# jlk9/MPAS-Ocean.jl

Measured on AMD Instinct MI355X. Metric: cell-updates/sec per RK4 step, higher is better.
Workload: dtype f64

## Files before the change

include/moka_hip.h:

```cpp
#ifndef MOKA_HIP_H
#define MOKA_HIP_H
#include <stdint.h>

#ifdef __cplusplus
extern "C" {
#endif

typedef struct moka_ctx   moka_ctx;
typedef struct moka_plan  moka_plan;
typedef struct moka_mesh  moka_mesh;
typedef struct moka_state moka_state;

typedef enum {
    MOKA_OK = 0,
    MOKA_ERR_ARG = -1,
    MOKA_ERR_HIP = -2,
    MOKA_ERR_NO_DEVICE = -3,
    MOKA_ERR_ALLOC = -4,
    MOKA_ERR_UNSUPPORTED = -5,
    MOKA_ERR_COMM = -6
} moka_status;

typedef enum {
    MOKA_ORDER_DEFAULT = 0,
    MOKA_ORDER_NONE = 1,
    MOKA_ORDER_RCM = 2,
    MOKA_ORDER_RCB = 3
} moka_ordering;

typedef struct moka_mesh_desc {
    int32_t nCells, nEdges, nVertices;
    int32_t maxEdges, maxEdges2, vertexDegree;
    int32_t nVertLevels;
    int32_t edgeSignOnVertexLD;
    const double  *xCell, *yCell, *zCell;
    const int32_t *nEdgesOnCell;
    const int32_t *edgesOnCell;
    const int32_t *edgeSignOnCell;
    const double  *areaCell;
    const int32_t *cellsOnEdge;
    const int32_t *verticesOnEdge;
    const int32_t *nEdgesOnEdge;
    const int32_t *edgesOnEdge;
    const double  *weightsOnEdge;
    const double  *dvEdge, *dcEdge, *fEdge;
    const int32_t *edgesOnVertex;
    const int32_t *cellsOnVertex;
    const int32_t *edgeSignOnVertex;
    const double  *areaTriangle;
    const int32_t *maxLevelEdgeTop;
    const double  *restingThicknessSum;
    int32_t ordering;
    int32_t patch_cells;
    const int32_t *cellClass;
    int32_t stateBytes;
    const double *kiteAreasOnVertex;
    const double *fVertex;
} moka_mesh_desc;

typedef struct moka_mesh_info {
    int32_t nCells, nEdges, nVertices, nVertLevels;
    int32_t ordering, patch_cells, nPatches;
    int32_t maxEdgesUsed, maxEdges2Used;
    int32_t lanesPerColumn;
    int64_t meshBytesDevice;
    int64_t cellBandwidth;
    int32_t maxPatchRows;
    int32_t ldsBytesPerBlock;
    int32_t maxPatchCells, maxPatchEdges;
} moka_mesh_info;

enum { MOKA_CELL = 0, MOKA_EDGE = 1, MOKA_VERTEX = 2 };

typedef enum {
    MOKA_F_SSH = 0,
    MOKA_F_NORMAL_VELOCITY = 1,
    MOKA_F_LAYER_THICKNESS = 2,
    MOKA_F_LAYER_THICKNESS_EDGE = 3,
    MOKA_F_THICKNESS_FLUX = 4,
    MOKA_F_VELOCITY_DIV_CELL = 5,
    MOKA_F_RELATIVE_VORTICITY = 6,
    MOKA_F_TEND_NORMAL_VELOCITY = 7,
    MOKA_F_TEND_LAYER_THICKNESS = 8
} moka_field;

#define MOKA_FE_STALE_HEDGE      1
#define MOKA_FE_ACCUM_VORT       2
#define MOKA_FE_LEVEL1_ONLY      4
#define MOKA_FE_REFERENCE_COMPAT 7

typedef enum { MOKA_FORWARD_EULER = 0, MOKA_RUNGE_KUTTA_4 = 1 } moka_integrator;

const char *moka_version(void);
int  moka_ctx_create(int device, moka_ctx **out);
void moka_ctx_destroy(moka_ctx *ctx);
const char *moka_last_error(const moka_ctx *ctx);
int  moka_sync(moka_ctx *ctx);
int  moka_timer_start(moka_ctx *ctx);
int  moka_timer_stop(moka_ctx *ctx, float *elapsed_ms);

int  moka_plan_create(const moka_mesh_desc *desc, moka_plan **out);
void moka_plan_destroy(moka_plan *plan);
int  moka_plan_info(const moka_plan *plan, moka_mesh_info *info);
int  moka_plan_permutation(const moka_plan *plan, int kind, int32_t *new_to_old);
int  moka_plan_patch_ranges(const moka_plan *plan, int32_t *cellStart, int32_t *edgeStart, int32_t *vertexStart);
int  moka_plan_class_ranges(const moka_plan *plan, int32_t capacity, int32_t *nClasses, int32_t *patchStart,
                            int32_t *cellStart, int32_t *edgeStart);

enum {
    MOKA_PA_EOC = 0, MOKA_PA_COC, MOKA_PA_MLTC, MOKA_PA_SDV, MOKA_PA_INVAREA, MOKA_PA_AREACELL, MOKA_PA_RSUM,
    MOKA_PA_EHDR, MOKA_PA_EOE, MOKA_PA_WOE, MOKA_PA_GINVDC, MOKA_PA_DCEDGE, MOKA_PA_DVEDGE, MOKA_PA_FEDGE,
    MOKA_PA_EOV, MOKA_PA_CV, MOKA_PA_HALO_START, MOKA_PA_HALO_EDGE, MOKA_PA_LEOC, MOKA_PA_LEOE,
    MOKA_PA_CREC, MOKA_PA_EREC, MOKA_PA_FEOE, MOKA_PA_PVSTART, MOKA_PA_PVLIST, MOKA_PA_LVOE
};
int  moka_plan_array(const moka_plan *plan, int which, const void **data, int64_t *count);

int  moka_mesh_create(moka_ctx *ctx, const moka_mesh_desc *desc, moka_mesh **out);
void moka_mesh_destroy(moka_mesh *mesh);
int  moka_mesh_info_get(const moka_mesh *mesh, moka_mesh_info *info);

int moka_gradient_on_edge(moka_mesh *mesh, const double *scalarCell, double *gradEdge);
int moka_divergence_on_cell(moka_mesh *mesh, const double *vecEdge, double *tempEdge, double *divCell);
int moka_curl_on_vertex(moka_mesh *mesh, const double *vecEdge, double *curlVertex);
int moka_interpolate_cell2edge(moka_mesh *mesh, const double *cellValue, double *edgeValue, int nlev);

int moka_gradient_on_edge_vjp(moka_mesh *mesh, double *dGradEdge , double *dScalarCell );
int moka_gradient_on_edge_jvp(moka_mesh *mesh, const double *dScalarCell, double *dGradEdge);
int moka_divergence_on_cell_vjp(moka_mesh *mesh, double *dDivCell , double *dVecEdge ,
                                double *dTempEdge );
int moka_divergence_on_cell_jvp(moka_mesh *mesh, const double *dVecEdge, double *dTempEdge , double *dDivCell);
int moka_curl_on_vertex_vjp(moka_mesh *mesh, const double *dCurlVertex, double *dVecEdge );
int moka_curl_on_vertex_jvp(moka_mesh *mesh, const double *dVecEdge, double *dCurlVertex );

int  moka_state_create(moka_ctx *ctx, moka_mesh *mesh, moka_state **out);
void moka_state_destroy(moka_state *st);
int  moka_state_upload(moka_state *st, int field, int time_level, const double *host);
int  moka_state_download(moka_state *st, int field, int time_level, double *host);

int  moka_state_download_rows(moka_state *st, int field, int time_level, int64_t nRows, const int32_t *rows, double *host);

int  moka_state_array_address(moka_state *st, int field, int time_level, uint64_t *address);

int  moka_state_optimize_placement(moka_state *st, int max_tries, double *ms_before, double *ms_after);
typedef struct { int32_t field; double ms_old, ms_new; int32_t kept; } moka_placement_trial;
int  moka_state_placement_log(const moka_state *st, int32_t capacity, moka_placement_trial *out, int32_t *n);
int64_t moka_state_placement_launches(const moka_state *st);

int moka_advance_time_levels(moka_state *st, int flags);
int moka_diagnostic_compute(moka_state *st, int flags);
int moka_compute_normal_velocity_tendency(moka_state *st, int flags);
int moka_compute_layer_thickness_tendency(moka_state *st, int flags);
int moka_tendencies(moka_state *st);
int moka_step_fe(moka_state *st, double dt, int flags);
int moka_step_rk4(moka_state *st, double dt);
int moka_run(moka_state *st, int integrator, double dt, int64_t nsteps, int flags);
int moka_sum_sq(moka_state *st, int field, int time_level, double *out);

typedef struct moka_halo moka_halo;
int  moka_ctx_streams(moka_ctx *ctx, void **compute_stream, void **comm_stream);
int  moka_mesh_permutation(const moka_mesh *mesh, int kind, int32_t *new_to_old);
int  moka_mesh_class_ranges(const moka_mesh *mesh, int32_t capacity, int32_t *nClasses, int32_t *patchStart,
                            int32_t *cellStart, int32_t *edgeStart);
int  moka_halo_create(moka_state *st, int32_t nNeighbors, const int32_t *sendCells, const int64_t *sendCellOff,
                      const int32_t *sendEdges, const int64_t *sendEdgeOff, const int32_t *recvCells,
                      const int64_t *recvCellOff, const int32_t *recvEdges, const int64_t *recvEdgeOff,
                      int32_t nPatchesBoundary, int32_t nPatchesOwned, moka_halo **out);
void moka_halo_destroy(moka_halo *h);
int  moka_halo_buffer_elems(const moka_halo *h, int64_t *sendElems, int64_t *recvElems);
int  moka_halo_pack(moka_halo *h, int what, void *sendbuf_device);
int  moka_halo_unpack(moka_halo *h, int what, const void *recvbuf_device);

typedef struct {
    unsigned char ipc[15][64];
    uint64_t ptr[15];
    uint64_t flagPtr;
    char     shmName[64];
    int32_t  dstCell, dstEdge;
    int32_t  nCells, nEdges;
    int32_t  slot;
    int32_t  nNeighbors, pid, device, stateBytes, nVertLevels;
// ... 104 lines not shown
```

mpas-ocean.jl_amd/csrc/plan.cpp:

```cpp
#include <algorithm>
#include <array>
#include <cmath>
#include <new>
#include <numeric>
#include <queue>

#include "moka_internal.hpp"

namespace moka {

static thread_local std::string g_err;
void set_error(const std::string &msg) { g_err = msg; }
const char *get_error() { return g_err.c_str(); }

namespace {

inline int64_t IX(int i, int64_t j, int ld) { return j * ld + i; }

#define REQUIRE(cond, msg)                 \
    do {                                   \
        if (!(cond)) {                     \
            set_error(msg);                \
            return MOKA_ERR_ARG;           \
        }                                  \
    } while (0)

std::vector<int> partition_by_class(const moka_mesh_desc *d, std::vector<int32_t> &n2o)
{
    std::vector<int> bounds{0};
    if (!d->cellClass) { bounds.push_back((int)n2o.size()); return bounds; }
    int maxc = 0;
    for (int c = 0; c < d->nCells; ++c) maxc = std::max(maxc, (int)d->cellClass[c]);
    std::vector<int32_t> out;
    out.reserve(n2o.size());
    for (int k = 0; k <= maxc; ++k) {
        for (int32_t c : n2o) if (d->cellClass[c] == k) out.push_back(c);
        bounds.push_back((int)out.size());
    }
    n2o.swap(out);
    return bounds;
}

void rcb_order(const moka_mesh_desc *d, int P, std::vector<int32_t> &n2o)
{
    const int n = d->nCells;
    n2o.resize(n);
    std::iota(n2o.begin(), n2o.end(), 0);
    const double *X[3] = {d->xCell, d->yCell, d->zCell};
    struct Range { int lo, hi; };
    std::vector<Range> stack;
    {
        const std::vector<int> b = partition_by_class(d, n2o);
        for (size_t i = b.size() - 1; i >= 1; --i) if (b[i] > b[i - 1]) stack.push_back({b[i - 1], b[i]});
    }
    while (!stack.empty()) {
        Range r = stack.back();
        stack.pop_back();
        const int cnt = r.hi - r.lo;
        if (cnt <= P) {
            continue;
        }
        int axis = 0;
        double best = -1.0;
        for (int a = 0; a < 3; ++a) {
            if (!X[a]) continue;
            double mn = 1e300, mx = -1e300;
            for (int i = r.lo; i < r.hi; ++i) {
                double v = X[a][n2o[i]];
                mn = std::min(mn, v);
                mx = std::max(mx, v);
            }
            if (mx - mn > best) { best = mx - mn; axis = a; }
        }
        const int leaves = (cnt + P - 1) / P;
        const int left = (leaves / 2) * P;
        const double *xa = X[axis];
        std::nth_element(n2o.begin() + r.lo, n2o.begin() + r.lo + left, n2o.begin() + r.hi,
                         [xa](int32_t a, int32_t b) { return xa[a] < xa[b] || (xa[a] == xa[b] && a < b); });
        stack.push_back({r.lo + left, r.hi});
        stack.push_back({r.lo, r.lo + left});
    }
}

void rcm_order(const moka_mesh_desc *d, std::vector<int32_t> &n2o)
{
    const int n = d->nCells;
    std::vector<int32_t> deg(n, 0), start(n + 1, 0), adj;
    for (int64_t e = 0; e < d->nEdges; ++e) {
        int a = d->cellsOnEdge[2 * e] - 1, b = d->cellsOnEdge[2 * e + 1] - 1;
        if (a >= 0 && b >= 0 && a != b) { ++deg[a]; ++deg[b]; }
    }
    for (int i = 0; i < n; ++i) start[i + 1] = start[i] + deg[i];
    adj.resize(start[n]);
    std::vector<int32_t> fill(start.begin(), start.end() - 1);
    for (int64_t e = 0; e < d->nEdges; ++e) {
        int a = d->cellsOnEdge[2 * e] - 1, b = d->cellsOnEdge[2 * e + 1] - 1;
        if (a >= 0 && b >= 0 && a != b) { adj[fill[a]++] = b; adj[fill[b]++] = a; }
    }
    std::vector<char> seen(n, 0);
    std::vector<int32_t> order;
    order.reserve(n);
    auto bfs_far = [&](int s, std::vector<int32_t> &lvl) {
        std::vector<int32_t> q{s};
        lvl.assign(n, -1);
        lvl[s] = 0;
        size_t h = 0;
        while (h < q.size()) {
            int u = q[h++];
            for (int k = start[u]; k < start[u + 1]; ++k)
                if (lvl[adj[k]] < 0 && !seen[adj[k]]) { lvl[adj[k]] = lvl[u] + 1; q.push_back(adj[k]); }
        }
        return q.back();
    };
    std::vector<int32_t> lvl;
    for (int s0 = 0; s0 < n; ++s0) {
        if (seen[s0]) continue;
        int s = bfs_far(bfs_far(s0, lvl), lvl);
        std::vector<int32_t> q{s};
        seen[s] = 1;
        size_t h = 0;
        std::vector<int32_t> nb;
        while (h < q.size()) {
            int u = q[h++];
            nb.clear();
            for (int k = start[u]; k < start[u + 1]; ++k)
                if (!seen[adj[k]]) { seen[adj[k]] = 1; nb.push_back(adj[k]); }
            std::sort(nb.begin(), nb.end(), [&](int a, int b) { return deg[a] < deg[b] || (deg[a] == deg[b] && a < b); });
            q.insert(q.end(), nb.begin(), nb.end());
        }
        order.insert(order.end(), q.begin(), q.end());
    }
    n2o.assign(order.rbegin(), order.rend());
}

}

int build_plan(const moka_mesh_desc *d, Plan &p)
{
    REQUIRE(d != nullptr, "mesh descriptor is NULL");
    REQUIRE(d->nCells > 0 && d->nEdges > 0 && d->nVertices > 0, "mesh counts must be positive");
    REQUIRE(d->nVertLevels >= 1, "nVertLevels must be >= 1");
    REQUIRE(d->maxEdges >= 3 && d->maxEdges2 >= 1 && d->vertexDegree >= 3, "bad maxEdges/maxEdges2/vertexDegree");
    REQUIRE(d->nEdgesOnCell && d->edgesOnCell && d->edgeSignOnCell && d->areaCell, "PrimaryCells arrays missing");
    REQUIRE(d->cellsOnEdge && d->nEdgesOnEdge && d->edgesOnEdge && d->weightsOnEdge && d->dvEdge && d->dcEdge && d->fEdge,
            "Edges arrays missing");
    REQUIRE(d->edgesOnVertex && d->edgeSignOnVertex && d->areaTriangle, "DualCells arrays missing");
    REQUIRE(d->restingThicknessSum, "restingThicknessSum missing");
    const int nC = d->nCells, nE = d->nEdges, nV = d->nVertices, VD = d->vertexDegree;
    const int ldSV = d->edgeSignOnVertexLD > 0 ? d->edgeSignOnVertexLD : VD;
    REQUIRE(ldSV >= VD, "edgeSignOnVertexLD < vertexDegree");

    int maxEoC = 0, maxEoE = 0;
    for (int c = 0; c < nC; ++c) {
        int n = d->nEdgesOnCell[c];
        REQUIRE(n >= 1 && n <= d->maxEdges, "nEdgesOnCell out of range");
        maxEoC = std::max(maxEoC, n);
        for (int i = 0; i < n; ++i) {
            int e = d->edgesOnCell[IX(i, c, d->maxEdges)];
            REQUIRE(e >= 1 && e <= nE, "edgesOnCell out of range");
            int s = d->edgeSignOnCell[IX(i, c, d->maxEdges)];
            REQUIRE(s == 1 || s == -1, "edgeSignOnCell must be +-1 on active slots");
        }
        REQUIRE(d->areaCell[c] > 0.0, "areaCell must be positive");
    }
    for (int e = 0; e < nE; ++e) {
        int a = d->cellsOnEdge[2 * (int64_t)e], b = d->cellsOnEdge[2 * (int64_t)e + 1];
        REQUIRE(a >= 1 && a <= nC && b >= 1 && b <= nC, "cellsOnEdge out of range (non-periodic meshes are not supported, VertMesh.jl:50)");
        int n = d->nEdgesOnEdge[e];
        REQUIRE(n >= 0 && n <= d->maxEdges2, "nEdgesOnEdge out of range");
        maxEoE = std::max(maxEoE, n);
        for (int i = 0; i < n; ++i) {
            int x = d->edgesOnEdge[IX(i, e, d->maxEdges2)];
            REQUIRE(x >= 0 && x <= nE, "edgesOnEdge out of range");
        }
        REQUIRE(d->dcEdge[e] > 0.0, "dcEdge must be positive");
        if (d->maxLevelEdgeTop) REQUIRE(d->maxLevelEdgeTop[e] >= 0 && d->maxLevelEdgeTop[e] <= d->nVertLevels, "maxLevelEdgeTop out of range");
    }
    for (int v = 0; v < nV; ++v) {
        for (int j = 0; j < VD; ++j) {
            int e = d->edgesOnVertex[IX(j, v, VD)];
            REQUIRE(e >= 1 && e <= nE, "edgesOnVertex out of range");
            int s = d->edgeSignOnVertex[IX(j, v, ldSV)];
            REQUIRE(s == 1 || s == -1, "edgeSignOnVertex must be +-1");
        }
        REQUIRE(d->areaTriangle[v] > 0.0, "areaTriangle must be positive");
    }

    p.nC = nC; p.nE = nE; p.nV = nV; p.K = d->nVertLevels; p.VD = VD;
    p.ME = maxEoC <= 6 ? 6 : (maxEoC <= 8 ? 8 : maxEoC);
    p.ME2 = maxEoE <= 10 ? 10 : (maxEoE <= 14 ? 14 : maxEoE);
    if (p.ME == 8 && p.ME2 < 14) p.ME2 = 14;
    {
        const int K = d->nVertLevels;
        REQUIRE(d->stateBytes == 0 || d->stateBytes == 4 || d->stateBytes == 8, "stateBytes must be 0, 4 or 8");
        p.stateBytes = d->stateBytes == 4 ? 4 : 8;
        int def = 32;
        if (p.stateBytes == 8 && K >= 34 && K <= 64 && !(K & 1)) def = 16;
        if (p.stateBytes == 4 && K >= 34 && K <= 128 && !(K & 3)) def = 24;
        p.P = d->patch_cells > 0 ? d->patch_cells : def;
    }
    REQUIRE(p.P <= 4096, "patch_cells too large");

    int ordering = d->ordering;
    const bool haveXYZ = d->xCell && d->yCell;
    if (ordering == MOKA_ORDER_DEFAULT) ordering = haveXYZ ? MOKA_ORDER_RCB : MOKA_ORDER_RCM;
    REQUIRE(ordering >= MOKA_ORDER_NONE && ordering <= MOKA_ORDER_RCB, "unknown ordering");
    REQUIRE(ordering != MOKA_ORDER_RCB || haveXYZ, "RCB ordering needs xCell/yCell");
    p.ordering = ordering;
    if (d->cellClass)
        for (int c = 0; c < nC; ++c) REQUIRE(d->cellClass[c] >= 0 && d->cellClass[c] < 64, "cellClass out of range");
    if (ordering == MOKA_ORDER_RCB) rcb_order(d, p.P, p.cellN2O);
    else if (ordering == MOKA_ORDER_RCM) { rcm_order(d, p.cellN2O); partition_by_class(d, p.cellN2O); }
    else { p.cellN2O.resize(nC); std::iota(p.cellN2O.begin(), p.cellN2O.end(), 0); partition_by_class(d, p.cellN2O); }
    p.cellO2N.assign(nC, -1);
    for (int i = 0; i < nC; ++i) p.cellO2N[p.cellN2O[i]] = i;

    std::vector<int32_t> patchOf(nC);
    p.classCellStart.assign(1, 0);
    p.classPatchStart.assign(1, 0);
    p.patchCellStart.assign(1, 0);
    {
        auto cls0 = [&](int cn) { return d->cellClass ? d->cellClass[p.cellN2O[cn]] : 0; };
        int begin = 0;
        while (begin < nC) {
            const int k = cls0(begin);
            int end = begin;
            while (end < nC && cls0(end) == k) ++end;
            REQUIRE((int)p.classCellStart.size() - 1 <= k, "internal: cell ordering is not class-major");
            while ((int)p.classCellStart.size() - 1 < k) {
                p.classCellStart.push_back(begin);
                p.classPatchStart.push_back((int)p.patchCellStart.size() - 1);
            }
            for (int c = begin; c < end; c += p.P) {
                const int q = (int)p.patchCellStart.size() - 1;
                for (int x = c; x < std::min(c + p.P, end); ++x) patchOf[x] = q;
                p.patchCellStart.push_back(std::min(c + p.P, end));
            }
            p.classCellStart.push_back(end);
            p.classPatchStart.push_back((int)p.patchCellStart.size() - 1);
            begin = end;
        }
    }
    p.nPatches = (int)p.patchCellStart.size() - 1;

    auto renumber = [&](int n, auto owner_of, std::vector<int32_t> &n2o, std::vector<int32_t> &o2n) {
        std::vector<int32_t> owner(n), cnt(nC + 1, 0);
        for (int i = 0; i < n; ++i) { owner[i] = owner_of(i); ++cnt[owner[i] + 1]; }
        for (int c = 0; c < nC; ++c) cnt[c + 1] += cnt[c];
        n2o.resize(n); o2n.resize(n);
        for (int i = 0; i < n; ++i) { int pos = cnt[owner[i]]++; n2o[pos] = i; o2n[i] = pos; }
        return owner;
    };
    std::vector<int32_t> ownerCell(nE);
    {
        const int P = p.P, nP = p.nPatches;
        std::vector<int32_t> cnt(nP, 0), flex;
        auto PO = [&](int cn) { return patchOf[cn]; };
        auto cls = [&](int cn) { return d->cellClass ? d->cellClass[p.cellN2O[cn]] : 0; };
        std::vector<int32_t> lo(nE), hi(nE);
        for (int e = 0; e < nE; ++e) {
            const int a = p.cellO2N[d->cellsOnEdge[2 * (int64_t)e] - 1], b = p.cellO2N[d->cellsOnEdge[2 * (int64_t)e + 1] - 1];
            lo[e] = std::min(a, b); hi[e] = std::max(a, b);
            if (PO(lo[e]) == PO(hi[e]) || cls(lo[e]) != cls(hi[e])) {
                ownerCell[e] = lo[e];
                ++cnt[PO(lo[e])];
            } else {
                ownerCell[e] = -1;
                flex.push_back(e);
            }
        }
        std::stable_sort(flex.begin(), flex.end(), [&](int x, int y) { return lo[x] < lo[y]; });
        for (int e : flex) {
            const int pa = PO(lo[e]), pb = PO(hi[e]);
            if (((uint32_t)e * 2654435761u >> 15) & 1u) { ownerCell[e] = lo[e]; ++cnt[pa]; }
            else { ownerCell[e] = hi[e]; ++cnt[pb]; }
        }
        for (int sweep = 0; sweep < 16; ++sweep) {
            int moved = 0;
            for (int e : flex) {
                const int cur = ownerCell[e], oth = cur == lo[e] ? hi[e] : lo[e];
                if (cnt[PO(cur)] > cnt[PO(oth)] + 1) { ownerCell[e] = oth; --cnt[PO(cur)]; ++cnt[PO(oth)]; ++moved; }
            }
            if (!moved) break;
        }
        {
            std::vector<int32_t> pcls(nP), Tc(64, 0);
            {
                std::vector<int64_t> tot(64, 0), num(64, 0);
                for (int q = 0; q < nP; ++q) {
                    pcls[q] = cls(p.patchCellStart[q]);
                    if (p.patchCellStart[q + 1] - p.patchCellStart[q] == P) { tot[pcls[q]] += cnt[q]; ++num[pcls[q]]; }
                }
                for (int c = 0; c < 64; ++c) Tc[c] = num[c] ? (int)((tot[c] + num[c] - 1) / num[c]) : 0;
            }
            auto T_of = [&](int q) { return Tc[pcls[q]]; };
            std::vector<int32_t> pstart(nP + 1, 0), plist;
            for (int e : flex) { ++pstart[PO(lo[e]) + 1]; ++pstart[PO(hi[e]) + 1]; }
            for (int q = 0; q < nP; ++q) pstart[q + 1] += pstart[q];
            plist.resize(pstart[nP]);
            {
                std::vector<int32_t> fill(pstart.begin(), pstart.end() - 1);
                for (int e : flex) { plist[fill[PO(lo[e])]++] = e; plist[fill[PO(hi[e])]++] = e; }
            }
            std::vector<int32_t> stamp(nP, -1), via(nP, -1), queue;
            int32_t tick = 0;
            for (int s = 0; s < nP; ++s) {
                for (int guard = 0; cnt[s] > T_of(s) && guard < 8; ++guard) {
                    queue.assign(1, s);
                    ++tick;
                    stamp[s] = tick; via[s] = -1;
                    int found = -1;
                    for (size_t h = 0; h < queue.size() && found < 0 && queue.size() < 2048; ++h) {
                        const int x = queue[h];
                        for (int k = pstart[x]; k < pstart[x + 1] && found < 0; ++k) {
                            const int e = plist[k];
                            if (PO(ownerCell[e]) != x) continue;
                            const int y = PO(ownerCell[e] == lo[e] ? hi[e] : lo[e]);
                            if (stamp[y] == tick) continue;
                            stamp[y] = tick; via[y] = e;
                            if (cnt[y] < T_of(y)) found = y;
                            else queue.push_back(y);
                        }
                    }
                    if (found < 0) break;
                    for (int y = found; y != s;) {
                        const int e = via[y];
                        const int x = PO(ownerCell[e]);
                        ownerCell[e] = ownerCell[e] == lo[e] ? hi[e] : lo[e];
                        --cnt[x]; ++cnt[y];
                        y = x;
                    }
                }
            }
        }
    }
    auto edgeOwner = renumber(nE, [&](int e) { return ownerCell[e]; }, p.edgeN2O, p.edgeO2N);
    auto vertOwner = renumber(nV, [&](int v) {
        int best = nC;
        for (int j = 0; j < VD; ++j) {
            if (d->cellsOnVertex) {
                int c = d->cellsOnVertex[IX(j, v, VD)];
                if (c >= 1 && c <= nC) best = std::min(best, (int)p.cellO2N[c - 1]);
            } else {
                int e = d->edgesOnVertex[IX(j, v, VD)] - 1;
                best = std::min(best, (int)p.cellO2N[d->cellsOnEdge[2 * (int64_t)e] - 1]);
                best = std::min(best, (int)p.cellO2N[d->cellsOnEdge[2 * (int64_t)e + 1] - 1]);
            }
        }
        return best == nC ? 0 : best;
    }, p.vertN2O, p.vertO2N);

    {
        std::vector<int32_t> ce(p.nPatches + 1, 0), cv(p.nPatches + 1, 0);
        for (int e = 0; e < nE; ++e) ++ce[patchOf[edgeOwner[e]] + 1];
        for (int v = 0; v < nV; ++v) ++cv[patchOf[vertOwner[v]] + 1];
        for (int q = 0; q < p.nPatches; ++q) { ce[q + 1] += ce[q]; cv[q + 1] += cv[q]; }
        p.patchEdgeStart = ce;
        p.patchVertStart = cv;
        p.classEdgeStart.resize(p.classPatchStart.size());
        for (size_t k = 0; k < p.classPatchStart.size(); ++k) p.classEdgeStart[k] = ce[p.classPatchStart[k]];
    }

    const int ME = p.ME, ME2 = p.ME2;
    p.eoc.assign((size_t)nC * ME, -1);
    p.coc.assign((size_t)nC * ME, -1);
    p.mltc.assign((size_t)nC * ME, 0);
    p.sdv.assign((size_t)nC * ME, 0.0);
    p.dvdc.assign((size_t)nC * ME, 0.0);
    p.invArea.resize(nC); p.areaCell.resize(nC); p.rsum.resize(nC);
    p.cellBandwidth = 0;
    for (int cn = 0; cn < nC; ++cn) {
        const int co = p.cellN2O[cn];
        const int n = d->nEdgesOnCell[co];
        for (int i = 0; i < n; ++i) {
            const int eo = d->edgesOnCell[IX(i, co, d->maxEdges)] - 1;
            const int a = d->cellsOnEdge[2 * (int64_t)eo] - 1, b = d->cellsOnEdge[2 * (int64_t)eo + 1] - 1;
            REQUIRE(a == co || b == co, "edgesOnCell / cellsOnEdge are inconsistent");
            const int other = (a == co) ? b : a;
            p.eoc[IX(i, cn, ME)] = p.edgeO2N[eo];
            p.coc[IX(i, cn, ME)] = p.cellO2N[other];
            p.mltc[IX(i, cn, ME)] = d->maxLevelEdgeTop ? d->maxLevelEdgeTop[eo] : 1;
            p.sdv[IX(i, cn, ME)] = d->dvEdge[eo] * (double)d->edgeSignOnCell[IX(i, co, d->maxEdges)];
            p.dvdc[IX(i, cn, ME)] = d->dvEdge[eo] / d->dcEdge[eo];
            p.cellBandwidth = std::max<int64_t>(p.cellBandwidth, std::abs((int64_t)p.cellO2N[other] - cn));
        }
        p.invArea[cn] = 1. / d->areaCell[co];
        p.areaCell[cn] = d->areaCell[co];
        p.rsum[cn] = d->restingThicknessSum[co];
    }
    p.ehdr.resize((size_t)nE * 4);
    p.eoe.assign((size_t)nE * ME2, -1);
    p.woe.assign((size_t)nE * ME2, 0.0);
    p.gInvDc.resize(nE); p.dcEdge.resize(nE); p.dvEdge.resize(nE); p.fEdge.resize(nE);
    for (int en = 0; en < nE; ++en) {
        const int eo = p.edgeN2O[en];
        const int n = d->nEdgesOnEdge[eo];
        p.ehdr[4 * (size_t)en + 0] = p.cellO2N[d->cellsOnEdge[2 * (int64_t)eo] - 1];
        p.ehdr[4 * (size_t)en + 1] = p.cellO2N[d->cellsOnEdge[2 * (int64_t)eo + 1] - 1];
        p.ehdr[4 * (size_t)en + 2] = n;
        p.ehdr[4 * (size_t)en + 3] = d->maxLevelEdgeTop ? d->maxLevelEdgeTop[eo] : 1;
        for (int i = 0; i < n; ++i) {
            const int x = d->edgesOnEdge[IX(i, eo, d->maxEdges2)];
            p.eoe[IX(i, en, ME2)] = x == 0 ? -1 : p.edgeO2N[x - 1];
            p.woe[IX(i, en, ME2)] = d->weightsOnEdge[IX(i, eo, d->maxEdges2)];
        }
        const double invDc = 1. / d->dcEdge[eo];
        p.gInvDc[en] = 9.80616 * invDc;
        p.dcEdge[en] = d->dcEdge[eo];
        p.dvEdge[en] = d->dvEdge[eo];
        p.fEdge[en] = d->fEdge[eo];
    }
    p.eov.resize((size_t)nV * VD);
    p.cv.resize((size_t)nV * VD);
    for (int vn = 0; vn < nV; ++vn) {
        const int vo = p.vertN2O[vn];
        const double invA = 1.0 / d->areaTriangle[vo];
        for (int j = 0; j < VD; ++j) {
            const int eo = d->edgesOnVertex[IX(j, vo, VD)] - 1;
            p.eov[IX(j, vn, VD)] = p.edgeO2N[eo];
            p.cv[IX(j, vn, VD)] = (d->dcEdge[eo] * invA) * (double)d->edgeSignOnVertex[IX(j, vo, ldSV)];
        }
    }
    p.nlOk = d->kiteAreasOnVertex && d->fVertex && d->verticesOnEdge && d->cellsOnVertex;
    if (p.nlOk) {
        p.voe.resize((size_t)nE * 2); p.cov.resize((size_t)nV * VD); p.kite.resize((size_t)nV * VD);
        p.invAreaTri.resize(nV); p.fVertex.resize(nV); p.keCoef.resize(nE); p.invDc.resize(nE);
        for (int en = 0; en < nE; ++en) {
            const int eo = p.edgeN2O[en];
            for (int q = 0; q < 2; ++q) {
                const int v = d->verticesOnEdge[2 * (int64_t)eo + q];
                REQUIRE(v >= 1 && v <= nV, "verticesOnEdge out of range");
                p.voe[(size_t)en * 2 + q] = p.vertO2N[v - 1];
            }
            p.keCoef[en] = 0.25 * d->dcEdge[eo] * d->dvEdge[eo];
            p.invDc[en] = 1. / d->dcEdge[eo];
        }
        for (int vn = 0; vn < nV; ++vn) {
            const int vo = p.vertN2O[vn];
            p.invAreaTri[vn] = 1.0 / d->areaTriangle[vo];
            p.fVertex[vn] = d->fVertex[vo];
            for (int j = 0; j < VD; ++j) {
                const int c = d->cellsOnVertex[IX(j, vo, VD)];
                REQUIRE(c >= 1 && c <= nC, "cellsOnVertex out of range");
                p.cov[IX(j, vn, VD)] = p.cellO2N[c - 1];
                p.kite[IX(j, vn, VD)] = d->kiteAreasOnVertex[IX(j, vo, VD)];
            }
        }
    }

    {
        const uint64_t rowB = (uint64_t)p.K * p.stateBytes;
        p.colOk = rowB * (uint64_t)std::max(nE, std::max(nC, nV)) < (1ull << 32) - 1024;
        p.CI = ((2 * ME + 2) + 3) & ~3;
        p.EI = ((ME2 + 4) + 3) & ~3;
        p.cRec.clear(); p.eRec.clear(); p.feoe.clear();
        if (p.colOk) {
            p.cRec.assign((size_t)nC * p.CI, 0u);
            p.eRec.assign((size_t)nE * p.EI, 0u);
            p.feoe.assign((size_t)nE * ME2, 0.0);
            for (int c = 0; c < nC; ++c) {
                uint32_t *r = &p.cRec[(size_t)c * p.CI];
                uint32_t mask = 0, all = 1;
                for (int i = 0; i < ME; ++i) {
                    const int e = p.eoc[IX(i, c, ME)];
                    if (e >= 0) {
                        mask |= 1u << i;
                        r[i] = (uint32_t)((uint64_t)e * rowB);
                        r[ME + i] = (uint32_t)((uint64_t)p.coc[IX(i, c, ME)] * rowB);
                        if (p.mltc[IX(i, c, ME)] < p.K) all = 0;
                    } else {
                        r[i] = (uint32_t)((uint64_t)p.eoc[IX(0, c, ME)] * rowB);
                        r[ME + i] = (uint32_t)((uint64_t)c * rowB);
                    }
                }
                r[2 * ME] = mask;
                r[2 * ME + 1] = all;
            }
            for (int e = 0; e < nE; ++e) {
                uint32_t *r = &p.eRec[(size_t)e * p.EI];
                uint32_t mask = 0;
                for (int i = 0; i < ME2; ++i) {
                    const int x = p.eoe[IX(i, e, ME2)];
                    if (x >= 0) {
                        mask |= 1u << i;
                        r[i] = (uint32_t)((uint64_t)x * rowB);
                        p.feoe[IX(i, e, ME2)] = p.fEdge[x];
                    } else {
// ... 235 lines not shown
```

mpas-ocean.jl_amd/moka_hip/lib.py:

```python
from __future__ import annotations

import ctypes as C
import os
import subprocess

import numpy as np

PKG_DIR = os.path.dirname(os.path.dirname(os.path.abspath(__file__)))
LIB_PATH = os.environ.get("MOKA_HIP_LIB") or os.path.join(PKG_DIR, "libmoka_hip.so")

_i32p = C.POINTER(C.c_int32)
_f64p = C.POINTER(C.c_double)

OK = 0
ERR_ARG, ERR_HIP, ERR_NO_DEVICE, ERR_ALLOC, ERR_UNSUPPORTED, ERR_COMM = -1, -2, -3, -4, -5, -6
ORDER_DEFAULT, ORDER_NONE, ORDER_RCM, ORDER_RCB = 0, 1, 2, 3
CELL, EDGE, VERTEX = 0, 1, 2
(F_SSH, F_NORMAL_VELOCITY, F_LAYER_THICKNESS, F_LAYER_THICKNESS_EDGE, F_THICKNESS_FLUX,
 F_VELOCITY_DIV_CELL, F_RELATIVE_VORTICITY, F_TEND_NORMAL_VELOCITY, F_TEND_LAYER_THICKNESS) = range(9)
FE_STALE_HEDGE, FE_ACCUM_VORT, FE_LEVEL1_ONLY, FE_REFERENCE_COMPAT = 1, 2, 4, 7
FORWARD_EULER, RUNGE_KUTTA_4 = 0, 1


class MokaError(RuntimeError):

    def __init__(self, code, msg):
        super().__init__(f"libmoka_hip error {code}: {msg}")
        self.code = code


class MeshDesc(C.Structure):
    _fields_ = [
        ("nCells", C.c_int32), ("nEdges", C.c_int32), ("nVertices", C.c_int32),
        ("maxEdges", C.c_int32), ("maxEdges2", C.c_int32), ("vertexDegree", C.c_int32),
        ("nVertLevels", C.c_int32), ("edgeSignOnVertexLD", C.c_int32),
        ("xCell", _f64p), ("yCell", _f64p), ("zCell", _f64p),
        ("nEdgesOnCell", _i32p), ("edgesOnCell", _i32p), ("edgeSignOnCell", _i32p), ("areaCell", _f64p),
        ("cellsOnEdge", _i32p), ("verticesOnEdge", _i32p), ("nEdgesOnEdge", _i32p), ("edgesOnEdge", _i32p),
        ("weightsOnEdge", _f64p), ("dvEdge", _f64p), ("dcEdge", _f64p), ("fEdge", _f64p),
        ("edgesOnVertex", _i32p), ("cellsOnVertex", _i32p), ("edgeSignOnVertex", _i32p), ("areaTriangle", _f64p),
        ("maxLevelEdgeTop", _i32p), ("restingThicknessSum", _f64p),
        ("ordering", C.c_int32), ("patch_cells", C.c_int32),
        ("cellClass", _i32p),
        ("stateBytes", C.c_int32),
        ("kiteAreasOnVertex", _f64p), ("fVertex", _f64p),
    ]


class HaloStats(C.Structure):
    _fields_ = [("steps", C.c_int64), ("exchanges", C.c_int64), ("boundary_launches", C.c_int64), ("interior_launches", C.c_int64),
                ("host_step_ms", C.c_double), ("host_signal_wait_ms", C.c_double), ("host_flag_store_ms", C.c_double),
                ("host_wait_ms", C.c_double), ("boundary_launch_ms", C.c_double), ("interior_launch_ms", C.c_double)]


class PlacementTrial(C.Structure):
    _fields_ = [("field", C.c_int32), ("ms_old", C.c_double), ("ms_new", C.c_double), ("kept", C.c_int32)]


class MeshInfo(C.Structure):
    _fields_ = [
        ("nCells", C.c_int32), ("nEdges", C.c_int32), ("nVertices", C.c_int32), ("nVertLevels", C.c_int32),
        ("ordering", C.c_int32), ("patch_cells", C.c_int32), ("nPatches", C.c_int32),
        ("maxEdgesUsed", C.c_int32), ("maxEdges2Used", C.c_int32), ("lanesPerColumn", C.c_int32),
        ("meshBytesDevice", C.c_int64), ("cellBandwidth", C.c_int64),
        ("maxPatchRows", C.c_int32), ("ldsBytesPerBlock", C.c_int32),
        ("maxPatchCells", C.c_int32), ("maxPatchEdges", C.c_int32),
    ]

    def as_dict(self):
        return {n: getattr(self, n) for n, _ in self._fields_}


EXPORTS = [
    "moka_version", "moka_ctx_create", "moka_ctx_destroy", "moka_last_error", "moka_sync",
    "moka_timer_start", "moka_timer_stop",
    "moka_plan_create", "moka_plan_destroy", "moka_plan_info", "moka_plan_permutation", "moka_plan_patch_ranges", "moka_plan_array",
    "moka_mesh_create", "moka_mesh_destroy", "moka_mesh_info_get",
    "moka_gradient_on_edge", "moka_divergence_on_cell", "moka_curl_on_vertex", "moka_interpolate_cell2edge",
    "moka_state_create", "moka_state_destroy", "moka_state_upload", "moka_state_download",
    "moka_advance_time_levels", "moka_diagnostic_compute", "moka_compute_normal_velocity_tendency",
    "moka_compute_layer_thickness_tendency", "moka_tendencies", "moka_step_fe", "moka_step_rk4", "moka_run",
    "moka_sum_sq", "moka_set_kernel_variant", "moka_kernel_variant_available", "moka_stage_timing", "moka_stage_timing_read",
    "moka_ctx_streams", "moka_halo_create", "moka_halo_destroy", "moka_halo_buffer_elems", "moka_halo_pack",
    "moka_halo_unpack", "moka_rk4_dist_begin", "moka_rk4_dist_stage", "moka_rk4_dist_end",
    "moka_plan_class_ranges", "moka_mesh_class_ranges", "moka_mesh_permutation", "moka_halo_direct_available", "moka_halo_set_overlap", "moka_halo_pack_fields", "moka_halo_unpack_fields",
    "moka_tape_record_rk4", "moka_tape_commit_rk4", "moka_adjoint_rk4_stage_fields", "moka_adjoint_rk4_stage",
    "moka_tape_record_fe", "moka_tape_commit_fe", "moka_adjoint_fe_step_fields", "moka_adjoint_fe_step",
    "moka_halo_export", "moka_halo_connect", "moka_halo_push_begin", "moka_halo_push_signal", "moka_halo_push_wait",
    "moka_rk4_dist_stage_launch", "moka_rk4_dist_step", "moka_fe_dist_launch", "moka_fe_dist_end", "moka_fe_dist_step",
    "moka_set_nonlinear", "moka_last_fe_path", "moka_set_viscosity_del2", "moka_set_viscosity_del4", "moka_state_del4_path", "moka_tape_create", "moka_tape_destroy", "moka_step_fe_taped", "moka_step_rk4_taped", "moka_adjoint_seed_sum_sq_ssh", "moka_adjoint_sweep",
    "moka_adjoint_download",
    "moka_mark", "moka_marks_reset", "moka_marks_read", "moka_bw_probe", "moka_bw_probe_streams", "moka_bw_probe_reread", "moka_bw_probe_gather_big", "moka_ctx_pci_bus_id", "moka_halo_set_acquire", "moka_set_tuning", "moka_get_tuning", "moka_rk4_dist_parts_available", "moka_adjoint_rk4_stage_part", "moka_adjoint_rk4_parts_available", "moka_adjoint_rk4_stage_out_fields",
    "moka_gradient_on_edge_vjp", "moka_gradient_on_edge_jvp", "moka_divergence_on_cell_vjp", "moka_divergence_on_cell_jvp",
    "moka_curl_on_vertex_vjp", "moka_curl_on_vertex_jvp", "moka_fe_lazy_pending",
    "moka_state_optimize_placement", "moka_state_placement_log", "moka_state_download_rows",
    "moka_halo_stats_enable", "moka_halo_stats_read", "moka_halo_set_stream_flags", "moka_state_array_address", "moka_state_placement_launches",
    "moka_state_rk4_streams",
    "moka_set_tracers", "moka_tracer_upload", "moka_tracer_download", "moka_state_tracer_path",
    "moka_set_tracer_diffusion", "moka_tracer_diffusion",
    "moka_tracer_source_upload", "moka_tracer_source_download", "moka_tracer_has_source",
    "moka_tracer_adjoint_want_source_gradient", "moka_tracer_adjoint_source_download",
    "moka_tracer_tape_create", "moka_tracer_tape_destroy", "moka_step_rk4_tracer_taped", "moka_tracer_tape_steps",
    "moka_tracer_adjoint_seed", "moka_tracer_adjoint_sweep", "moka_tracer_adjoint_download", "moka_tracer_adjoint_path",
]


def build(force: bool = False) -> str:
    if force:
        subprocess.check_call(["make", "-C", PKG_DIR, "--no-print-directory", "clean"])
    subprocess.check_call(["make", "-C", PKG_DIR, "--no-print-directory", "-j4"])
    return LIB_PATH


_lib = None


def lib():
    global _lib
    if _lib is not None:
        return _lib
    if not os.path.exists(LIB_PATH):
        raise MokaError(ERR_NO_DEVICE, f"{LIB_PATH} is missing: build it with `make -C {PKG_DIR}` "
                                       "(there is no CPU fallback for the HIP path)")
    try:
        import torch
    except ImportError:
        pass
    L = C.CDLL(LIB_PATH)
    vp = C.c_void_p
    L.moka_version.restype = C.c_char_p
    L.moka_last_error.restype = C.c_char_p
    L.moka_last_error.argtypes = [vp]
    L.moka_ctx_create.argtypes = [C.c_int, C.POINTER(vp)]
    L.moka_ctx_destroy.argtypes = [vp]
    L.moka_ctx_destroy.restype = None
    L.moka_sync.argtypes = [vp]
    L.moka_timer_start.argtypes = [vp]
    L.moka_timer_stop.argtypes = [vp, C.POINTER(C.c_float)]
    L.moka_plan_create.argtypes = [C.POINTER(MeshDesc), C.POINTER(vp)]
    L.moka_plan_destroy.argtypes = [vp]
    L.moka_plan_destroy.restype = None
    L.moka_plan_info.argtypes = [vp, C.POINTER(MeshInfo)]
    L.moka_plan_permutation.argtypes = [vp, C.c_int, _i32p]
    L.moka_plan_patch_ranges.argtypes = [vp, _i32p, _i32p, _i32p]
    L.moka_plan_array.argtypes = [vp, C.c_int, C.POINTER(vp), C.POINTER(C.c_int64)]
    L.moka_mesh_create.argtypes = [vp, C.POINTER(MeshDesc), C.POINTER(vp)]
    L.moka_mesh_destroy.argtypes = [vp]
    L.moka_mesh_destroy.restype = None
    L.moka_mesh_info_get.argtypes = [vp, C.POINTER(MeshInfo)]
    L.moka_gradient_on_edge.argtypes = [vp, _f64p, _f64p]
    L.moka_divergence_on_cell.argtypes = [vp, _f64p, _f64p, _f64p]
    L.moka_curl_on_vertex.argtypes = [vp, _f64p, _f64p]
    L.moka_interpolate_cell2edge.argtypes = [vp, _f64p, _f64p, C.c_int]
    L.moka_gradient_on_edge_vjp.argtypes = [vp, _f64p, _f64p]
    L.moka_gradient_on_edge_jvp.argtypes = [vp, _f64p, _f64p]
    L.moka_divergence_on_cell_vjp.argtypes = [vp, _f64p, _f64p, _f64p]
    L.moka_divergence_on_cell_jvp.argtypes = [vp, _f64p, _f64p, _f64p]
    L.moka_curl_on_vertex_vjp.argtypes = [vp, _f64p, _f64p]
    L.moka_curl_on_vertex_jvp.argtypes = [vp, _f64p, _f64p]
    L.moka_state_create.argtypes = [vp, vp, C.POINTER(vp)]
    L.moka_state_destroy.argtypes = [vp]
    L.moka_state_destroy.restype = None
    L.moka_state_optimize_placement.argtypes = [vp, C.c_int, _f64p, _f64p]
    L.moka_state_placement_launches.argtypes = [vp]
    L.moka_state_rk4_streams.argtypes = [vp]
    L.moka_state_placement_launches.restype = C.c_int64
    L.moka_state_placement_log.argtypes = [vp, C.c_int32, C.POINTER(PlacementTrial), _i32p]
    L.moka_state_array_address.argtypes = [vp, C.c_int, C.c_int, C.POINTER(C.c_uint64)]
    L.moka_state_download_rows.argtypes = [vp, C.c_int, C.c_int, C.c_int64, _i32p, _f64p]
# ... 242 lines not shown
```

Baseline: 9.051 billion.

## Refine edge ownership between patches to reduce cross-patch halo edges

Adds a plan-time refinement pass that reassigns flexible inter-patch edges between their two adjacent patches. For each patch pair it uses exhaustive bitmask search on small boundaries, and boundary-ordered contiguous splits on larger ones, to minimise the number of external edge-on-edge neighbours each patch must fetch. Fewer out-of-patch neighbours should mean less redundant halo loading in the patch kernels. It adds host setup cost and a new RCB_UNREFINED ordering option that keeps the old behaviour; refinement also runs under the RCM and NONE orderings.

```diff
diff --git a/include/moka_hip.h b/include/moka_hip.h
--- a/include/moka_hip.h
+++ b/include/moka_hip.h
@@ -25,7 +25,8 @@
     MOKA_ORDER_DEFAULT = 0,
     MOKA_ORDER_NONE = 1,
     MOKA_ORDER_RCM = 2,
-    MOKA_ORDER_RCB = 3
+    MOKA_ORDER_RCB = 3,
+    MOKA_ORDER_RCB_UNREFINED = 4
 } moka_ordering;
 
 typedef struct moka_mesh_desc {
diff --git a/mpas-ocean.jl_amd/csrc/plan.cpp b/mpas-ocean.jl_amd/csrc/plan.cpp
--- a/mpas-ocean.jl_amd/csrc/plan.cpp
+++ b/mpas-ocean.jl_amd/csrc/plan.cpp
@@ -1,5 +1,6 @@
 #include <algorithm>
 #include <array>
+#include <climits>
 #include <cmath>
 #include <new>
 #include <numeric>
@@ -133,6 +134,233 @@
     n2o.assign(order.rbegin(), order.rend());
 }
 
+void refine_ownership(const moka_mesh_desc *d, int nP, const std::vector<int32_t> &patchOf, const std::vector<int32_t> &lo,
+                      const std::vector<int32_t> &hi, const std::vector<int32_t> &flex, std::vector<int32_t> &ownerCell)
+{
+    constexpr int kExhaustive = 12, kSweeps = 8, kBits = 128;
+    const int nE = d->nEdges, LD = d->maxEdges2;
+    if (flex.empty()) return;
+    std::vector<int32_t> tstart(nP + 1, 0), e2t(nE), t2e(nE), pl(nE), ph(nE);
+    std::vector<char> ownHi(nE), isFlex(nE, 0);
+    for (int e = 0; e < nE; ++e) ++tstart[patchOf[lo[e]] + 1];
+    for (int q = 0; q < nP; ++q) tstart[q + 1] += tstart[q];
+    {
+        std::vector<int32_t> fill(tstart.begin(), tstart.end() - 1);
+        for (int e = 0; e < nE; ++e) {
+            const int t = fill[patchOf[lo[e]]]++;
+            e2t[e] = t; t2e[t] = e;
+            pl[t] = patchOf[lo[e]]; ph[t] = patchOf[hi[e]];
+            ownHi[t] = ownerCell[e] != lo[e];
+        }
+    }
+    for (int e : flex) isFlex[e2t[e]] = 1;
+    auto owner = [&](int t) { return ownHi[t] ? ph[t] : pl[t]; };
+    auto incident = [&](int t, int q) { return pl[t] == q || ph[t] == q; };
+    std::vector<int32_t> xid(nE, -1), xeoe, xstart(nP + 1, 0), xlist;
+    xeoe.reserve(2 * flex.size() * LD);
+    for (int t = 0; t < nE; ++t) {
+        if (pl[t] == ph[t]) continue;
+        const int e = t2e[t];
+        const int32_t *r = &d->edgesOnEdge[(int64_t)e * LD];
+        const int n = d->nEdgesOnEdge[e];
+        xid[t] = (int32_t)(xeoe.size() / LD);
+        for (int i = 0; i < LD; ++i) xeoe.push_back(i < n && r[i] > 0 ? e2t[r[i] - 1] : -1);
+        ++xstart[pl[t] + 1];
+        if (ph[t] != pl[t]) ++xstart[ph[t] + 1];
+    }
+    for (int q = 0; q < nP; ++q) xstart[q + 1] += xstart[q];
+    xlist.resize(xstart[nP]);
+    {
+        std::vector<int32_t> fill(xstart.begin(), xstart.end() - 1);
+        for (int t = 0; t < nE; ++t) {
+            if (xid[t] < 0) continue;
+            xlist[fill[pl[t]]++] = t;
+            if (ph[t] != pl[t]) xlist[fill[ph[t]]++] = t;
+        }
+    }
+    auto eoe_of = [&](int t) { return &xeoe[(size_t)xid[t] * LD]; };
+    std::vector<int32_t> side;
+    side.reserve(flex.size());
+    for (int q = 0; q < nP; ++q) {
+        const size_t b = side.size();
+        for (int t = tstart[q]; t < tstart[q + 1]; ++t) if (isFlex[t]) side.push_back(t);
+        std::sort(side.begin() + b, side.end(), [&](int x, int y) { return ph[x] != ph[y] ? ph[x] < ph[y] : x < y; });
+    }
+    std::vector<int32_t> stQ(nE, 0), stR(nE, 0), stS(nE, 0), flipped(nE, 0), lastEval(side.size(), 0);
+    int32_t tick = 0;
+    auto stamp_base = [&](int q, std::vector<int32_t> &st) {
+        for (int j = xstart[q]; j < xstart[q + 1]; ++j) {
+            const int x = xlist[j];
+            if (owner(x) != q || stS[x] == tick) continue;
+            const int32_t *r = eoe_of(x);
+            for (int i = 0; i < LD; ++i)
+                if (r[i] >= 0) st[r[i]] = tick;
+        }
+    };
+    std::vector<int32_t> locQ, locR, offQ, offR, idsQ, idsR, seen;
+    auto candidates = [&](int t, int q, std::vector<int32_t> &st, std::vector<int32_t> &loc, std::vector<int32_t> &ids) {
+        const int32_t *r = eoe_of(t);
+        for (int i = 0; i < LD; ++i) {
+            const int y = r[i];
+            if (y < 0 || st[y] == tick || incident(y, q)) continue;
+            if (st[y] >= 0) { st[y] = -(int32_t)loc.size() - 1; loc.push_back(y); }
+            ids.push_back(-st[y] - 1);
+        }
+    };
+    std::vector<char> toQ, best;
+    auto cost_of = [&](const std::vector<char> &sel) {
+        int c = 0;
+        seen.assign(locQ.size() + locR.size(), 0);
+        for (size_t i = 0; i < sel.size(); ++i) {
+            const std::vector<int32_t> &off = sel[i] ? offQ : offR, &ids = sel[i] ? idsQ : idsR;
+            const int base = sel[i] ? 0 : (int)locQ.size();
+            for (int j = off[i]; j < off[i + 1]; ++j)
+                if (!seen[base + ids[j]]) { seen[base + ids[j]] = 1; ++c; }
+        }
+        return c;
+    };
+    std::vector<int32_t> ev, vst, vfirst, order;
+    auto boundary_order = [&](const int32_t *S, int s) {
+        if (ev.empty()) {
+            ev.assign((size_t)nE * 2, -1);
+            for (int v = 0; v < d->nVertices; ++v)
+                for (int j = 0; j < d->vertexDegree; ++j) {
+                    const int t = e2t[d->edgesOnVertex[(int64_t)v * d->vertexDegree + j] - 1];
+                    if (ev[2 * (size_t)t] < 0) ev[2 * (size_t)t] = v;
+                    else if (ev[2 * (size_t)t + 1] < 0) ev[2 * (size_t)t + 1] = v;
+                }
+            vst.assign(d->nVertices, 0);
+            vfirst.assign(d->nVertices, -1);
+        }
+        std::vector<int32_t> nb(2 * (size_t)s, -1);
+        auto link = [&](int a, int b) {
+            for (int k = 0; k < 2; ++k) if (nb[2 * a + k] < 0) { nb[2 * a + k] = b; return; }
+        };
+        for (int i = 0; i < s; ++i)
+            for (int k = 0; k < 2; ++k) {
+                const int v = ev[2 * (size_t)S[i] + k];
+                if (v < 0) continue;
+                if (vst[v] == tick) { link(i, vfirst[v]); link(vfirst[v], i); }
+                else { vst[v] = tick; vfirst[v] = i; }
+            }
+        order.clear();
+        std::vector<char> done(s, 0);
+        for (int pass = 0; pass < 2; ++pass)
+            for (int i0 = 0; i0 < s; ++i0) {
+                if (done[i0] || (pass == 0 && nb[2 * i0] >= 0 && nb[2 * i0 + 1] >= 0)) continue;
+                for (int i = i0; i >= 0 && !done[i];) {
+                    done[i] = 1;
+                    order.push_back(i);
+                    const int a = nb[2 * i], b = nb[2 * i + 1];
+                    i = (a >= 0 && !done[a]) ? a : (b >= 0 && !done[b]) ? b : -1;
+                }
+            }
+    };
+
+    for (int sweep = 0; sweep < kSweeps && tick < INT32_MAX - 2 * (int64_t)side.size() - 2; ++sweep) {
+        int moved = 0;
+        for (size_t s0 = 0, s1; s0 < side.size(); s0 = s1) {
+            const int q = pl[side[s0]], r = ph[side[s0]];
+            for (s1 = s0 + 1; s1 < side.size() && pl[side[s1]] == q && ph[side[s1]] == r;) ++s1;
+            const int32_t *S = &side[s0];
+            const int s = (int)(s1 - s0);
+            int k = 0;
+            for (int i = 0; i < s; ++i) k += !ownHi[S[i]];
+            if (k == 0 || k == s) continue;
+            if (sweep > 0) {
+                bool stale = false, stamped = false;
+                for (int side_of = 0; side_of < 2 && !stale; ++side_of) {
+                    const int w = side_of ? r : q;
+                    for (int j = xstart[w]; j < xstart[w + 1] && !stale; ++j) {
+                        const int x = xlist[j];
+                        if (flipped[x] <= lastEval[s0]) continue;
+                        if (!stamped) {
+                            ++tick;
+                            for (int i = 0; i < s; ++i) {
+                                const int32_t *e = eoe_of(S[i]);
+                                for (int m = 0; m < LD; ++m) if (e[m] >= 0) stS[e[m]] = tick;
+                            }
+                            stamped = true;
+                        }
+                        const int32_t *e = eoe_of(x);
+                        for (int m = 0; m < LD; ++m) if (e[m] >= 0 && stS[e[m]] == tick && !incident(e[m], w)) { stale = true; break; }
+                    }
+                }
+                if (!stale) continue;
+            }
+            ++tick;
+            lastEval[s0] = tick;
+            for (int i = 0; i < s; ++i) stS[S[i]] = tick;
+            stamp_base(q, stQ);
+            stamp_base(r, stR);
+            locQ.clear(); locR.clear(); idsQ.clear(); idsR.clear();
+            offQ.assign(1, 0); offR.assign(1, 0);
+            for (int i = 0; i < s; ++i) {
+                candidates(S[i], q, stQ, locQ, idsQ); offQ.push_back((int32_t)idsQ.size());
+                candidates(S[i], r, stR, locR, idsR); offR.push_back((int32_t)idsR.size());
+            }
+            for (int y : locQ) stQ[y] = 0;
+            for (int y : locR) stR[y] = 0;
+            if (locQ.empty() && locR.empty()) continue;
+            toQ.resize(s);
+            for (int i = 0; i < s; ++i) toQ[i] = !ownHi[S[i]];
+            best = toQ;
+            if (s <= kExhaustive && (int)locQ.size() <= kBits && (int)locR.size() <= kBits) {
+                uint64_t mq[kExhaustive][2] = {}, mr[kExhaustive][2] = {};
+                for (int i = 0; i < s; ++i) {
+                    for (int j = offQ[i]; j < offQ[i + 1]; ++j) mq[i][idsQ[j] >> 6] |= 1ull << (idsQ[j] & 63);
+                    for (int j = offR[i]; j < offR[i + 1]; ++j) mr[i][idsR[j] >> 6] |= 1ull << (idsR[j] & 63);
+                }
+                constexpr int kHalf = kExhaustive / 2;
+                const int nl = (s + 1) / 2, nh = s - nl;
+                uint64_t tq[2][1 << kHalf][2], tr[2][1 << kHalf][2];
+                for (int h = 0; h < 2; ++h) {
+                    tq[h][0][0] = tq[h][0][1] = tr[h][0][0] = tr[h][0][1] = 0;
+                    for (int m = 1; m < 1 << (h ? nh : nl); ++m) {
+                        const int i = __builtin_ctz(m) + (h ? nl : 0), rest = m & (m - 1);
+                        for (int w = 0; w < 2; ++w) { tq[h][m][w] = tq[h][rest][w] | mq[i][w]; tr[h][m][w] = tr[h][rest][w] | mr[i][w]; }
+                    }
+                }
+                auto cost = [&](uint32_t A) {
+                    const uint32_t al = A & ((1u << nl) - 1), ah = A >> nl, bl = ~A & ((1u << nl) - 1), bh = (~A >> nl) & ((1u << nh) - 1);
+                    return __builtin_popcountll(tq[0][al][0] | tq[1][ah][0]) + __builtin_popcountll(tq[0][al][1] | tq[1][ah][1]) +
+                           __builtin_popcountll(tr[0][bl][0] | tr[1][bh][0]) + __builtin_popcountll(tr[0][bl][1] | tr[1][bh][1]);
+                };
+                uint32_t cur = 0;
+                for (int i = 0; i < s; ++i) cur |= (uint32_t)toQ[i] << i;
+                uint32_t bestA = cur;
+                int bestC = cost(cur);
+                for (uint32_t A = (1u << k) - 1; A < (1u << s);) {
+                    const int c = cost(A);
+                    if (c < bestC) { bestC = c; bestA = A; }
+                    const uint32_t low = A & (~A + 1), up = A + low;
+                    A = (((up ^ A) >> 2) / low) | up;
+                }
+                for (int i = 0; i < s; ++i) best[i] = bestA >> i & 1u;
+            } else {
+                boundary_order(S, s);
+                int bestC = cost_of(toQ);
+                std::vector<char> cand(s);
+                for (int end = 0; end < 2; ++end) {
+                    std::fill(cand.begin(), cand.end(), 0);
+                    for (int j = 0; j < k; ++j) cand[order[end ? s - 1 - j : j]] = 1;
+                    const int c = cost_of(cand);
+                    if (c < bestC) { bestC = c; best = cand; }
+                }
+            }
+            if (best == toQ) continue;
+            for (int i = 0; i < s; ++i) {
+                if (best[i] == toQ[i]) continue;
+                ownHi[S[i]] = !best[i];
+                flipped[S[i]] = tick;
+            }
+            ++moved;
+        }
+        if (!moved) break;
+    }
+    for (int e : flex) ownerCell[e] = ownHi[e2t[e]] ? hi[e] : lo[e];
+}
+
 }
 
 int build_plan(const moka_mesh_desc *d, Plan &p)
@@ -204,9 +432,11 @@
     int ordering = d->ordering;
     const bool haveXYZ = d->xCell && d->yCell;
     if (ordering == MOKA_ORDER_DEFAULT) ordering = haveXYZ ? MOKA_ORDER_RCB : MOKA_ORDER_RCM;
-    REQUIRE(ordering >= MOKA_ORDER_NONE && ordering <= MOKA_ORDER_RCB, "unknown ordering");
+    REQUIRE(ordering >= MOKA_ORDER_NONE && ordering <= MOKA_ORDER_RCB_UNREFINED, "unknown ordering");
+    p.ordering = ordering;
+    const bool refineOwnership = ordering != MOKA_ORDER_RCB_UNREFINED;
+    if (!refineOwnership) ordering = MOKA_ORDER_RCB;
     REQUIRE(ordering != MOKA_ORDER_RCB || haveXYZ, "RCB ordering needs xCell/yCell");
-    p.ordering = ordering;
     if (d->cellClass)
         for (int c = 0; c < nC; ++c) REQUIRE(d->cellClass[c] >= 0 && d->cellClass[c] < 64, "cellClass out of range");
     if (ordering == MOKA_ORDER_RCB) rcb_order(d, p.P, p.cellN2O);
@@ -333,6 +563,7 @@
                 }
             }
         }
+        if (refineOwnership) refine_ownership(d, nP, patchOf, lo, hi, flex, ownerCell);
     }
     auto edgeOwner = renumber(nE, [&](int e) { return ownerCell[e]; }, p.edgeN2O, p.edgeO2N);
     auto vertOwner = renumber(nV, [&](int v) {
diff --git a/mpas-ocean.jl_amd/moka_hip/lib.py b/mpas-ocean.jl_amd/moka_hip/lib.py
--- a/mpas-ocean.jl_amd/moka_hip/lib.py
+++ b/mpas-ocean.jl_amd/moka_hip/lib.py
@@ -14,7 +14,7 @@
 
 OK = 0
 ERR_ARG, ERR_HIP, ERR_NO_DEVICE, ERR_ALLOC, ERR_UNSUPPORTED, ERR_COMM = -1, -2, -3, -4, -5, -6
-ORDER_DEFAULT, ORDER_NONE, ORDER_RCM, ORDER_RCB = 0, 1, 2, 3
+ORDER_DEFAULT, ORDER_NONE, ORDER_RCM, ORDER_RCB, ORDER_RCB_UNREFINED = 0, 1, 2, 3, 4
 CELL, EDGE, VERTEX = 0, 1, 2
 (F_SSH, F_NORMAL_VELOCITY, F_LAYER_THICKNESS, F_LAYER_THICKNESS_EDGE, F_THICKNESS_FLUX,
  F_VELOCITY_DIV_CELL, F_RELATIVE_VORTICITY, F_TEND_NORMAL_VELOCITY, F_TEND_LAYER_THICKNESS) = range(9)
```

Measured after the change: 9.145 billion, median of 6. 1.0% higher.
